# JuliaMeshless/WhatsThePoint.jl

Measured on AMD Instinct MI355X. Metric: Mpoints/sec per repel iter (k=21 KNN+force), higher is better.
Workload: dtype f32

## Files before the change

### whatsthepoint.jl_amd/csrc/wtp_cs2.hip

```cpp
#include "wtp_device.hpp"

namespace wtp {

#ifndef WTP_DIAG
#define WTP_DIAG 0
#endif
#define CS_STAMP(i)                                                 \
    if (WTP_DIAG) {                                                 \
        const unsigned long long t_ = __builtin_amdgcn_s_memtime(); \
        dt[i] += t_ - t_last;                                       \
        t_last = t_;                                                \
    }

constexpr int kCsThreads = 256;
constexpr int kCsSlab = 16;
constexpr int kCsMaxBX = 61;
constexpr int kCsMaxCells = (kCsMaxBX + 2) * kCsSlab;
constexpr int kCsMaskSteps = 12;
constexpr int kCsSU = 8;
constexpr int kCsPadBytes = 2 * kCsSU * 16;
constexpr int kCsMaxQ = 512;
constexpr int kCsMiss = 16;
constexpr int kCsRun = 2 * kCsSlab + 2 * 4 + 3;

struct CsMiss {
    uint32_t pa, ea, qoff;
    int32_t gslot, qid;
    float f, s, g2;
};

struct Cs2Smem {
    uint32_t hglobal[kCsMaxCells];
    uint16_t ls[kCsMaxCells + 4];
    uint16_t qpref[kCsMaxBX + 2];
    uint8_t qslab[kCsMaxQ];
    uint32_t wsum[4][64], wcnt[4][64], wown[2][64];
    int scan_tmp[kCsThreads / 64 + 1];
    int miss_n[kCsThreads / 64];
    CsMiss miss[kCsThreads / 64][kCsMiss];
    Acc acc[kCsThreads / 64];
};

struct CsAcc {
    float max_force, argmin_r;
    double sum_u, sum_u2;
    int32_t argmin_i, argmin_j, n_move;
};
__device__ inline float cs_step_point(const SearchArgs<float>& a, float s, float xi, float yi, float zi, float Fx, float Fy,
                                      float Fz, float& xo, float& yo, float& zo) {
    const float Fn = __builtin_amdgcn_sqrtf((Fx * Fx + Fy * Fy) + Fz * Fz);
    float al = __builtin_amdgcn_rcpf(Fn + 1.0e-30f);
// ... 10 lines not shown
}

__device__ inline void cs_acc_point(CsAcc& c, float force, float nd, float s, int32_t id, int32_t nn) {
    c.max_force = force > c.max_force ? force : c.max_force;
    const float rs = __builtin_amdgcn_rcpf(s), q0 = nd * rs;
    const double u = (double)__builtin_fmaf(__builtin_fmaf(-s, q0, nd), rs, q0);
    c.sum_u += u;
    c.sum_u2 += u * u;
    c.n_move += 1;
    if (nd < c.argmin_r || (nd == c.argmin_r && id < c.argmin_i)) {
        c.argmin_r = nd;
        c.argmin_i = id;
        c.argmin_j = nn;
    }
}

struct ForceCoefCs {
    float A, beta;
};
__device__ inline ForceCoefCs force_coef_cs(float beta, float u0) { return ForceCoefCs{u0 * u0, beta}; }

static size_t cs2_smem_bytes(int hcap) {
    return (size_t)hcap * 16 + kCsPadBytes + sizeof(Cs2Smem);
}

template <bool CH>
__global__ __launch_bounds__(kCsThreads, 4) void cs2_kernel(SearchArgs<float> a, int hcap, int BX) {
    if (a.stop && *a.stop) return;
    extern __shared__ __attribute__((aligned(16))) unsigned char smem_raw[];
    float4* pts = reinterpret_cast<float4*>(smem_raw);
    Cs2Smem* sm = reinterpret_cast<Cs2Smem*>(smem_raw + (size_t)hcap * 16 + kCsPadBytes);
    const int tid = threadIdx.x, lane = tid & 63;
    const int wave = __builtin_amdgcn_readfirstlane(tid >> 6);

    const Grid<float> g = *a.grid;
    const int K = a.k;
    const int HX = BX + 2, ncell = HX * kCsSlab;
    const int nbx = (g.n[0] + BX - 1) / BX, nby = (g.n[1] + 1) / 2, nbz = (g.n[2] + 1) / 2;
    const int nbricks = nbx * nby * nbz;
    CsAcc acc;
    acc.max_force = 0.f;
    acc.argmin_r = Lim<float>::inf();
    acc.sum_u = acc.sum_u2 = 0.0;
    acc.argmin_i = acc.argmin_j = -1;
    acc.n_move = 0;
    unsigned long long dt[16] = {0, 0, 0, 0, 0, 0, 0, 0, 0, 0, 0, 0, 0, 0, 0, 0};
// ... 47 lines not shown
            const int r = wave * 4 + j;
            const int gy = oy + (r & 3), gz = oz + (r >> 2);
            const bool row_ok = gy >= 0 && gy < g.n[1] && gz >= 0 && gz < g.n[2];
            vv[j] = a.cell_start[row_ok ? (gz * g.n[1] + gy) * g.n[0] + gxc : 0];
        }
    };
    auto load_points = [&](const int (&vv)[4], float4 (&pp)[4]) {
        const int last = a.n - 1;
#pragma unroll
        for (int j = 0; j < 4; ++j) {
            const int gs = __builtin_amdgcn_readfirstlane(vv[j]);
            const int len = __builtin_amdgcn_readlane(vv[j], HX < 63 ? HX : 63) - gs;
            const int i = gs + (lane < len ? lane : 0);
            pp[j] = a.snap[i < last ? i : last];
        }
    };

    auto skip_dead = [&](int& b, BrickPos& p) {
        while (a.brick_dead && b < b_end && b < a.brick_dead_cap && a.brick_dead[b]) {
            b += blk_per_group;
            advance(p);
        }
    };
    int brick = xcd * per + lane_blk;
    BrickPos pos = brick_pos(brick < nbricks ? brick : 0);
    skip_dead(brick, pos);
    BrickPos pos_next = pos;
    int next = brick;
    int v[4] = {0, 0, 0, 0};
    float4 pv[4];
    pv[0] = pv[1] = pv[2] = pv[3] = make_float4(0.f, 0.f, 0.f, 0.f);
    if (brick < b_end) {
        load_cells(pos, v);
        load_points(v, pv);
    }
    for (; brick < b_end; brick = next, pos = pos_next) {
        int bx, ox, oy, oz;
        origin(pos, bx, ox, oy, oz);
        next = brick + blk_per_group;
        advance(pos_next);
        skip_dead(next, pos_next);

        __builtin_amdgcn_s_setprio(0);
        __syncthreads();
        int vn[4] = {0, 0, 0, 0};
        if (next < b_end) load_cells(pos_next, vn);
// ... 320 lines not shown
            a.forces[gslot] = f;
            const bool has = nid != 0x7FFFFFFF;
            if (has) {
                const float nd = wsqrt(nd2);
                if (reaches_past_cover<float>(a, qp.x, qp.y, qp.z, lim)) atomicAdd(a.uncovered, 1);
                a.nn_dist[gslot] = nd;
                a.nn_id[gslot] = nid;
                cs_acc_point(acc, f, nd, s, qid, nid);
            }
            const unsigned long long mm = __ballot(!has);
            if (mm) {
                const int base_m = sm->miss_n[wave];
                if (!has) {
                    const int pos = base_m + (int)__popcll(mm & ((1ull << lane) - 1ull));
                    if (pos < kCsMiss) {
                        CsMiss e;
                        e.pa = pa_first;
                        e.ea = ea_all;
                        e.qoff = qoff;
                        e.gslot = gslot;
                        e.qid = qid;
                        e.f = f;
                        e.s = s;
                        e.g2 = safe_radius2(g, qp.x, qp.y, qp.z, cx, cy, cz, 1);
                        sm->miss[wave][pos] = e;
                    } else {
                        const int p2 = atomicAdd(a.fb_count, 1);
                        a.fb_list[p2] = gslot;
                    }
                }
                const int first = __ffsll((long long)mm) - 1;
                const int tot = base_m + (int)__popcll(mm);
                __builtin_amdgcn_wave_barrier();
                if (lane == first) sm->miss_n[wave] = tot < kCsMiss ? tot : kCsMiss;
                __builtin_amdgcn_wave_barrier();
            }
            CS_STAMP(4)
        }

        {
            const int nm = __builtin_amdgcn_readfirstlane(sm->miss_n[wave]);
            for (int m = 0; m < nm; ++m) {
                const CsMiss e = sm->miss[wave][m];
                const float4 qp = lds_pt(smem_raw, e.qoff);
                float bd = Lim<float>::inf();
                int32_t bi = 0x7FFFFFFF;
                for (uint32_t p = e.pa + (uint32_t)lane * 16u; p < e.ea; p += 64u * 16u) {
                    const float4 c = lds_pt(smem_raw, p);
                    const int32_t cid = w_to_id(c.w);
                    const float d = dist2<float>(qp.x, qp.y, qp.z, c.x, c.y, c.z);
                    if (cid != e.qid && lex_lt(d, cid, bd, bi)) {
                        bd = d;
                        bi = cid;
                    }
                }
#pragma unroll
                for (int dlt = 32; dlt >= 1; dlt >>= 1) {
                    const float od = __shfl_xor(bd, dlt, 64);
                    const int32_t oi = __shfl_xor(bi, dlt, 64);
                    if (lex_lt(od, oi, bd, bi)) {
                        bd = od;
                        bi = oi;
                    }
                }
                if (lane == 0) {
                    if (bi != 0x7FFFFFFF && bd <= e.g2) {
                        const float nd = wsqrt(bd);
                        if (reaches_past_cover<float>(a, qp.x, qp.y, qp.z, bd)) atomicAdd(a.uncovered, 1);
                        a.nn_dist[e.gslot] = nd;
                        a.nn_id[e.gslot] = bi;
                        cs_acc_point(acc, e.f, nd, e.s, e.qid, bi);
                    } else {
                        a.nn_dist[e.gslot] = bd;
                        a.nn_id[e.gslot] = bi == 0x7FFFFFFF ? -1 : bi;
                        const int pos = atomicAdd(a.nn_count, 1);
                        a.nn_list[pos] = e.gslot;
                    }
                }
            }
            if (WTP_DIAG) dt[14] += (unsigned long long)nm;
        }
        CS_STAMP(5)
    }
    if (WTP_DIAG && a.diag && lane == 0) {
        for (int i = 0; i < 15; ++i) atomicAdd(&a.diag[i], dt[i]);
        atomicAdd(&a.diag[15], 1ull);
    }
    __syncthreads();
    Acc full = acc_empty();
    full.max_force = (double)acc.max_force;
    full.sum_u = acc.sum_u;
    full.sum_u2 = acc.sum_u2;
    full.n_move = acc.n_move;
    if (acc.argmin_i >= 0) {
        full.argmin_r = (double)acc.argmin_r;
        full.argmin_i = acc.argmin_i;
        full.argmin_j = acc.argmin_j;
    }
    acc_block_reduce(full, sm->acc);
    if (tid == 0) acc_store(&a.partials[blockIdx.x], full);
}

__global__ void cs2_census_kernel(const int32_t* __restrict__ cell_start, const Grid<float>* __restrict__ gp, int BX,
                                  unsigned int* __restrict__ out ) {
    const Grid<float> g = *gp;
    const int nbx = (g.n[0] + BX - 1) / BX, nby = (g.n[1] + 1) / 2, nbz = (g.n[2] + 1) / 2;
    const int nbricks = nbx * nby * nbz;
    for (int brick = blockIdx.x * blockDim.x + threadIdx.x; brick < nbricks; brick += gridDim.x * blockDim.x) {
        const int bx = brick % nbx, by = (brick / nbx) % nby, bz = brick / (nbx * nby);
// ... 5 lines not shown
            if (gy < 0 || gy >= g.n[1] || gz < 0 || gz >= g.n[2]) continue;
            const int base = (gz * g.n[1] + gy) * g.n[0];
            H += cell_start[base + hx1 + 1] - cell_start[base + hx0];
            const bool own = ((r & 3) == 1 || (r & 3) == 2) && ((r >> 2) == 1 || (r >> 2) == 2);
            if (own) Q += cell_start[base + gx1 + 1] - cell_start[base + gx0];
        }
        if (Q == 0) continue;
        atomicAdd(&out[Q / 2 < 255 ? Q / 2 : 255], 1u);
        atomicAdd(&out[256 + (H / 8 < 255 ? H / 8 : 255)], 1u);
        atomicAdd(&out[512], 1u);
    }
}

int launch_cs2_census(wtp_ctx* ctx, int BX, unsigned int* d_out513) {
    WTP_HIP(ctx, hipMemsetAsync(d_out513, 0, 513 * sizeof(unsigned int), ctx->stream));
    hipLaunchKernelGGL(cs2_census_kernel, dim3(512), dim3(256), 0, ctx->stream, (const int32_t*)ctx->cell_start.p,
                       (const Grid<float>*)ctx->grid.p, BX, d_out513);
    WTP_HIP(ctx, hipGetLastError());
    return WTP_OK;
}

int cs2_max_bx() { return kCsMaxBX; }

constexpr int kNnFixBlocks = 512;
constexpr int kNnFixThreads = 1024;
__global__ __launch_bounds__(kNnFixThreads, 8) void cs2_nnfix_kernel(SearchArgs<float> a, int part_base) {
    if (a.stop && *a.stop) return;
    __shared__ Acc sacc[kNnFixThreads / 64];
    const Grid<float> g = *a.grid;
    const int n = *a.nn_count;
    const int lane = threadIdx.x & 63;
    const int wave_g = (blockIdx.x * kNnFixThreads + threadIdx.x) >> 6, nwaves = (gridDim.x * kNnFixThreads) >> 6;
    Acc acc = acc_empty();
    const int grp = lane >> 4, l16 = lane & 15;
    for (int i0 = wave_g * 4; i0 < n; i0 += nwaves * 4) {
        const int i = i0 + grp;
        const bool on = i < n;
        const int gslot = a.nn_list[on ? i : i0];
        const float4 qp = a.snap[gslot];
        const int32_t qid = w_to_id(qp.w);
        const int cx = cell_coord(g, qp.x, 0), cy = cell_coord(g, qp.y, 1), cz = cell_coord(g, qp.z, 2);
        float bd = a.nn_dist[gslot];
        int32_t bi = a.nn_id[gslot];
        bi = bi < 0 ? 0x7FFFFFFF : bi;
        auto gap = [&](float v, int axis, int c, int lo, int hi) {
            const float a0 = g.org[axis] + (float)(c + lo) * g.c, a1 = g.org[axis] + (float)(c + hi + 1) * g.c;
            float d = v < a0 ? a0 - v : (v > a1 ? v - a1 : 0.f);
            d -= g.margin;
            return d > 0.f ? d : 0.f;
        };
        for (int piece = l16; piece < 75; piece += 16) {
            const int r = piece / 3, seg = piece % 3;
            const int dz = r / 5 - 2, dy = r % 5 - 2;
            const bool inner = dz >= -1 && dz <= 1 && dy >= -1 && dy <= 1;
            if (inner && seg == 1) continue;
            const int gz = cz + dz, gy = cy + dy;
            if (gz < 0 || gz >= g.n[2] || gy < 0 || gy >= g.n[1]) continue;
            int xa = seg == 0 ? cx - 2 : (seg == 1 ? cx - 1 : cx + 2), xb = seg == 1 ? cx + 1 : xa;
            xa = xa < 0 ? 0 : xa;
            xb = xb > g.n[0] - 1 ? g.n[0] - 1 : xb;
            if (xa > xb) continue;
            const bool edge = xa == 0 || xb == g.n[0] - 1 || gy == 0 || gy == g.n[1] - 1 || gz == 0 || gz == g.n[2] - 1;
            if (!edge) {
                const float gx2 = gap(qp.x, 0, 0, xa, xb), gy2 = gap(qp.y, 1, gy, 0, 0), gz2 = gap(qp.z, 2, gz, 0, 0);
                if ((gx2 * gx2 + gy2 * gy2) + gz2 * gz2 > bd) continue;
            }
            const int base = (gz * g.n[1] + gy) * g.n[0];
            const int p1 = a.cell_start[base + xb + 1];
            for (int p = a.cell_start[base + xa]; p < p1; p += 4) {
                float4 c[4];
#pragma unroll
                for (int u = 0; u < 4; ++u) c[u] = a.snap[p + u < p1 ? p + u : p];
#pragma unroll
                for (int u = 0; u < 4; ++u) {
                    const int32_t cid = w_to_id(c[u].w);
                    const float d = dist2<float>(qp.x, qp.y, qp.z, c[u].x, c[u].y, c[u].z);
                    if (p + u < p1 && cid != qid && lex_lt(d, cid, bd, bi)) {
                        bd = d;
                        bi = cid;
                    }
                }
            }
        }
#pragma unroll
        for (int dlt = 8; dlt >= 1; dlt >>= 1) {
            const float od = __shfl_xor(bd, dlt, 64);
            const int32_t oi = __shfl_xor(bi, dlt, 64);
            if (lex_lt(od, oi, bd, bi)) {
                bd = od;
                bi = oi;
            }
        }
        if (l16 == 0 && on) {
            const float g2 = safe_radius2(g, qp.x, qp.y, qp.z, cx, cy, cz, 2);
            if (bi != 0x7FFFFFFF && bd <= g2) {
                const float s = a.spacing_pp ? a.spacing_pp[qid] : a.spacing_const;
                const float nd = wsqrt(bd);
                if (reaches_past_cover<float>(a, qp.x, qp.y, qp.z, bd)) atomicAdd(a.uncovered, 1);
                a.nn_dist[gslot] = nd;
                a.nn_id[gslot] = bi;
                acc_point<float>(acc, a.forces[gslot], nd, s, qid, bi);
            } else {
                const int pos = atomicAdd(a.fb_count, 1);
                a.fb_list[pos] = gslot;
            }
        }
    }
    acc_block_reduce(acc, sacc);
    if (threadIdx.x == 0) acc_store(&a.partials[part_base + blockIdx.x], acc);
}

constexpr int kBallThreads = 256;
constexpr int kBallBlocksMax = 3072;
constexpr int kBallRMax = 4;
#ifndef WTP_BALL_LANES
#define WTP_BALL_LANES 8
#endif
constexpr int kBallLanes = WTP_BALL_LANES;
constexpr int kBallPerWave = 64 / kBallLanes;
__global__ __launch_bounds__(kBallThreads, 6) void cs_ball_kernel(SearchArgs<float> a, const int32_t* __restrict__ list,
                                                               const int32_t* __restrict__ list_count,
                                                               int32_t* __restrict__ out_list, int32_t* __restrict__ out_count,
                                                               int part_base) {
    if (a.stop && *a.stop) return;
    __shared__ Acc sacc[kBallThreads / 64];
    const Grid<float> g = *a.grid;
    const int n = *list_count;
    const int K = a.k;
    const int lane = threadIdx.x & 63;
    const int grp = lane / kBallLanes, l16 = lane % kBallLanes;
    const int wave_g = (blockIdx.x * kBallThreads + threadIdx.x) >> 6, nwaves = (gridDim.x * kBallThreads) >> 6;
    const ForceCoef fc = force_coef(WTP_FORCE_CLIPPED_SPACING, a.beta, a.u0, 0.f);
    Acc acc = acc_empty();
// ... 170 lines not shown
    return WTP_OK;
}

int launch_cs2(wtp_ctx* ctx, SearchArgs<float>& a) {
    const int hcap = a.brick_hcap, BX = a.cs2_bx;
    if (hcap < 64 || hcap > 4096 || BX < 1 || BX > kCsMaxBX)
        return fail(ctx, WTP_ERR_STATE, "compact-support sweep launched without a brick geometry");
    const size_t smem = cs2_smem_bytes(hcap);
    const bool chunked = a.cs2_chunked != 0;
    const void* fn = chunked ? (const void*)cs2_kernel<true> : (const void*)cs2_kernel<false>;
    if (ctx->cs2_smem != smem || ctx->cs2_fn != fn) {
        WTP_HIP(ctx, hipFuncSetAttribute(fn, hipFuncAttributeMaxDynamicSharedMemorySize, (int)smem));
        int occ = 0;
        hipError_t e = chunked ? hipOccupancyMaxActiveBlocksPerMultiprocessor(&occ, cs2_kernel<true>, kCsThreads, smem)
                               : hipOccupancyMaxActiveBlocksPerMultiprocessor(&occ, cs2_kernel<false>, kCsThreads, smem);
        if (e != hipSuccess || occ < 1) occ = 1;
        ctx->cs2_occ = occ > 4 ? 4 : occ;
        ctx->cs2_smem = smem;
        ctx->cs2_fn = fn;
    }
    int gsz = ctx->sm_count * ctx->cs2_occ;
    gsz -= gsz % 8;
    if (gsz < 8) gsz = 8;
    if (chunked)
        hipLaunchKernelGGL(cs2_kernel<true>, dim3(gsz), dim3(kCsThreads), smem, ctx->stream, a, hcap, BX);
    else
        hipLaunchKernelGGL(cs2_kernel<false>, dim3(gsz), dim3(kCsThreads), smem, ctx->stream, a, hcap, BX);
    a.used_brick = gsz;
    WTP_HIP(ctx, hipGetLastError());
    return WTP_OK;
}

int launch_cs2_followup(wtp_ctx* ctx, SearchArgs<float>& a) {
    int blocks = (int)((a.n + 2047) / 2048);
    blocks = blocks < 8 ? 8 : (blocks > kNnFixBlocks ? kNnFixBlocks : blocks);
    hipLaunchKernelGGL(cs2_nnfix_kernel, dim3(blocks), dim3(kNnFixThreads), 0, ctx->stream, a, a.used_brick);
    a.used_brick += blocks;
    WTP_HIP(ctx, hipGetLastError());
    return WTP_OK;
}

}
```

### whatsthepoint.jl_amd/csrc/wtp_device.hpp

```cpp
#pragma once
#include "wtp_internal.hpp"

namespace wtp {

template <typename T> struct Lim;
template <> struct Lim<float> {
    static __device__ __host__ constexpr float inf() { return __builtin_huge_valf(); }
};
template <> struct Lim<double> {
    static __device__ __host__ constexpr double inf() { return __builtin_huge_val(); }
};

__device__ inline float wsqrt(float x) { return __builtin_sqrtf(x); }
__device__ inline double wsqrt(double x) { return __builtin_sqrt(x); }
__device__ inline float wfloor(float x) { return floorf(x); }
__device__ inline double wfloor(double x) { return floor(x); }
__device__ inline float wpow(float a, float b) { return powf(a, b); }
__device__ inline double wpow(double a, double b) { return pow(a, b); }

template <typename T>
__device__ inline T dist2(T ax, T ay, T az, T bx, T by, T bz) {
    T dx = ax - bx;
    T dy = ay - by;
    T dz = az - bz;
// ... 10 lines not shown
template <typename T>
__device__ inline int cell_coord(const Grid<T>& g, T v, int axis) {
    T f = wfloor((v - g.org[axis]) * g.inv_c);
    int c = (f > (T)0) ? ((f < (T)(g.n[axis] - 1)) ? (int)f : g.n[axis] - 1) : 0;
    return c;
}

template <typename T>
__device__ inline T safe_radius2(const Grid<T>& g, T qx, T qy, T qz, int cx, int cy, int cz, int r) {
    T best = Lim<T>::inf();
    const T q[3] = {qx, qy, qz};
    const int c[3] = {cx, cy, cz};
#pragma unroll
    for (int a = 0; a < 3; ++a) {
        if (a >= g.dim) break;
        T rel = q[a] - g.org[a];
        if (c[a] - r > 0) {
            T lo = rel - (T)(c[a] - r) * g.c;
            best = lo < best ? lo : best;
        }
        if (c[a] + r < g.n[a] - 1) {
            T hi = (T)(c[a] + r + 1) * g.c - rel;
            best = hi < best ? hi : best;
        }
    }
    if (best == Lim<T>::inf()) return best;
    best = best - g.margin;
    if (best < (T)0) best = (T)0;
    return best * best;
}

template <typename T>
__device__ inline T force_law(int kind, T beta, T u0, T gamma, T u) {
    T u2 = u * u;
    T d = u2 + beta;
    if (kind == WTP_FORCE_INVERSE_DISTANCE) return (T)1 / (d * d);
    if (kind == WTP_FORCE_SPACING_EQUILIBRIUM) return ((T)1 - u2) / (d * d);
    if (kind == WTP_FORCE_CLIPPED_SPACING) {
        T f = (u0 * u0 - u2) / (d * d);
        return f > (T)0 ? f : (T)0;
    }
    return ((T)1 - u2) / wpow(d, gamma);
}

template <typename T>
__device__ inline void fallback_dir(int64_t i, int64_t j, int dim, T out[3]) {
// ... 257 lines not shown
```

### whatsthepoint.jl_amd/csrc/wtp_generic.hip

```cpp
#include "wtp_device.hpp"

namespace wtp {

static constexpr int kThreads = 128;

template <typename T, int MODE>
__global__ __launch_bounds__(kThreads) void generic_kernel(SearchArgs<T> a, const int32_t* __restrict__ list,
                                                           const int32_t* __restrict__ list_count,
                                                           int all, int part_base) {
    if (a.stop && *a.stop) return;
    __shared__ Acc sm_acc[kThreads / 64];
    const Grid<T> g = *a.grid;
    const int nq = all ? a.n : *list_count;
    const int K = a.k;
    const bool skip_self = (MODE == 0) && !a.include_self;
    T bd[kGenericKMax];
    int32_t bi[kGenericKMax];
    int32_t bp[kGenericKMax];
    Acc acc = acc_empty();

    for (int qi = blockIdx.x * blockDim.x + threadIdx.x; qi < nq; qi += gridDim.x * blockDim.x) {
        const int slot = all ? qi : list[qi];
        const Pt<T> q = a.query[slot];
        const int32_t id = w_to_id(q.w);
        if (MODE == 1 && id < a.n_fixed) {
            a.out[slot] = q;
            a.forces[slot] = (T)0;
            a.nn_dist[slot] = Lim<T>::inf();
            a.nn_id[slot] = -1;
            continue;
        }
        const int cx = cell_coord(g, q.x, 0), cy = cell_coord(g, q.y, 1), cz = cell_coord(g, q.z, 2);
        int m = 0;
        for (int r = 1;; r *= 2) {
            m = 0;
            const int z0 = cz - r < 0 ? 0 : cz - r, z1 = cz + r > g.n[2] - 1 ? g.n[2] - 1 : cz + r;
// ... 260 lines not shown
```

### whatsthepoint.jl_amd/csrc/wtp_internal.hpp

```cpp
#pragma once
#include <hip/hip_runtime.h>
#include <stddef.h>
#include <stdint.h>
#include <functional>
#include <map>
#include <string>
#include <utility>
#include <vector>

#include "../../include/wtp.h"

namespace wtp {

template <typename T> struct PtOf;
template <> struct PtOf<float> { using type = float4; };
template <> struct PtOf<double> { using type = double4; };
template <typename T> using Pt = typename PtOf<T>::type;

using KnnStats = struct ::wtp_knn_stats;

template <typename F> inline auto by_dtype(int dtype, F&& f) { return dtype == WTP_F32 ? f(float{}) : f(double{}); }

__host__ __device__ inline float id_to_w(float, int32_t id) { return __builtin_bit_cast(float, id); }
__host__ __device__ inline double id_to_w(double, int32_t id) {
// ... 32 lines not shown
int brick_partials();
constexpr int kGenericKMax = 128;

constexpr double kGammaCap = 1.0;
constexpr double kGammaCapSweep = 0.96;
constexpr double kTnnFrac = 0.8;
constexpr double kRhoCs2 = 1.0;
constexpr double kRhoKsel = 1.2;
constexpr double kCapKsel = 40.0;
constexpr int kGridReuseMax = 7;

struct Partial {
    double max_force;
    double sum_u;
    double sum_u2;
    double argmin_r;
    int64_t argmin_i;
    int64_t argmin_j;
    int64_t n_move;
};

struct StepCounters {
    int32_t brick_handbacks, pad1_;
    int32_t nn_count, pad3_;
    int32_t wave_handbacks, pad5_;
    int32_t ball_count, pad7_;
    int32_t uncovered, pad9_[3];
    int32_t escaped, pad13_[3];
};
static_assert(sizeof(StepCounters) == 64 && offsetof(StepCounters, escaped) == 48, "16 words: the reduction zeroes exactly these");

struct RadCursor {
    unsigned long long arena_next;
    int32_t bricks_listed;
    int32_t dense_queries;
};
static_assert(sizeof(RadCursor) == 16, "wtp_radb.hip addresses these words by offset");

struct ForceParams {
    int32_t kind;
    double beta, u0, gamma;
};

template <typename T> struct SearchArgs {
    const Grid<T>* grid;
    const Pt<T>* snap;
    const int32_t* cell_start;
// ... 13 lines not shown
    T beta, u0, gamma;
    int32_t force_kind;
    int32_t n_fixed;
    Partial* partials;
    int32_t n_partials;
    int32_t used_brick, used_wave, used_generic;
    T radius2;
    int32_t* rad_counts;
    const int64_t* rad_offsets;
    int32_t rad_fill;
    int32_t* rad_tmp;
    uint8_t* rad_done;
    int32_t* rad_arena;
    int64_t* rad_arena_off;
    unsigned long long* rad_arena_pos;
    int64_t rad_arena_cap;
    int32_t* rad_bricks;
    int32_t rad_dense;
    int32_t* fb_list;
    int32_t* fb_count;
    int32_t* fb2_list;
    int32_t* fb2_count;
    int32_t* nn_list;
    int32_t* nn_count;
    int32_t* ball_list;
    int32_t* ball_count;
    const int32_t* stop;
    int32_t cover_axis;
    T cover_lo, cover_hi;
    T cover_lo3[3], cover_hi3[3];
    int32_t* uncovered;
    T gamma_cap;
    float cap_count;
    T tnn_frac;
    int32_t brick_hcap;
    int32_t cs2_bx;
    const uint8_t* brick_dead;
    int32_t brick_dead_cap;
    int32_t cs2_chunked;
    int32_t counters_cleared;
    int32_t fb_r0;
    int32_t ksel_bx;
    unsigned long long* diag;
};

struct DevBuf {
    void* p = nullptr;
// ... 341 lines not shown

inline int grid_for(int64_t n, int threads, int cap) {
    int64_t b = (n + threads - 1) / threads;
    if (b < 1) b = 1;
    return (int)(b > cap ? cap : b);
}
template <typename T> int launch_topology(wtp_ctx* ctx, SearchArgs<T>& a);
int launch_brick_sweep(wtp_ctx* ctx, SearchArgs<float>& a, bool cs);
template <typename T> int launch_brick_cs(wtp_ctx* ctx, SearchArgs<T>& a);
template <typename T> int launch_wave_topology(wtp_ctx* ctx, SearchArgs<T>& a, bool all);
template <typename T> int launch_wave_sweep(wtp_ctx* ctx, SearchArgs<T>& a, bool all);
template <typename T>
int launch_wave_radius_count(wtp_ctx* ctx, SearchArgs<T>& a, T r, int32_t* d_counts, const int32_t* list,
                             const int32_t* list_count);
template <typename T>
int launch_wave_radius_fill(wtp_ctx* ctx, SearchArgs<T>& a, T r, const int64_t* d_offsets, int32_t* d_idx,
                            const int32_t* list, const int32_t* list_count);
template <typename T> int launch_generic_topology(wtp_ctx* ctx, SearchArgs<T>& a, bool all);
template <typename T> int launch_query_knn(wtp_ctx* ctx, SearchArgs<T>& a, const T* d_xyz, int dim, Pt<T>* d_packed);
template <typename T> int launch_generic_sweep(wtp_ctx* ctx, SearchArgs<T>& a, bool all);
inline int total_partials() { return brick_partials() + kWavePartials + kGenericPartials; }
int launch_brick_radius(wtp_ctx* ctx, SearchArgs<float>& a);
int launch_cs2(wtp_ctx* ctx, SearchArgs<float>& a);
int launch_cs2_followup(wtp_ctx* ctx, SearchArgs<float>& a);
int debug_kd_steps(unsigned long long out[2]);
int launch_cs_ball(wtp_ctx* ctx, SearchArgs<float>& a, int32_t* rest_list, int32_t* rest_count);
int launch_cs2_census(wtp_ctx* ctx, int BX, unsigned int* d_out513);
int launch_cs2_dead(wtp_ctx* ctx, SearchArgs<float>& a, uint8_t* d_dead, int dead_cap);
int cs2_max_bx();
int launch_ksel_topology(wtp_ctx* ctx, SearchArgs<float>& a);
int launch_ksel_sweep(wtp_ctx* ctx, SearchArgs<float>& a);
int ksel_max_bx();
int ksel_kmax();
template <typename T>
int launch_radius_count(wtp_ctx* ctx, SearchArgs<T>& a, T r, int32_t* d_counts);
template <typename T>
int launch_radius_fill(wtp_ctx* ctx, SearchArgs<T>& a, T r, const int64_t* d_offsets,
                       int32_t* d_idx);
int launch_reduce_partials(wtp_ctx* ctx, const Partial* parts, int n_parts, int used_brick, int used_wave,
                           int used_generic, const int32_t* fb_count, const int32_t* uncovered,
                           const int32_t* escaped, wtp_step_stats* d_stats_slot);
template <typename T>
int launch_pca_normals(wtp_ctx* ctx, const T* d_xyz, int64_t n, int dim, const int32_t* d_rows, int k, T* d_out);
template <typename T>
int launch_minplus_batch(wtp_ctx* ctx, const int32_t* d_rows, const T* d_dist, int64_t n, int k, double g, double tol,
                         T* d_h0, T* d_h1, int first, int sweeps, unsigned long long* d_state);
size_t knn_stats_tmp_bytes(int64_t n);
template <typename T>
int launch_knn_stats(wtp_ctx* ctx, const T* d_dist, int64_t n, int k, const double* d_h, double h_const, int has_spacing,
                     double coord_radius, const int64_t* d_gid, T* d_nn_out, double* d_mean_out, void* d_tmp,
                     const KnnStats** d_result_out, const unsigned long long** d_bad_out);
int knn_stats_spacing(const void* h, double h_const, double coord_radius, const char** why);
// ... 84 lines not shown
```

### whatsthepoint.jl_amd/csrc/wtp_relax.hip

```cpp
#include <cstdlib>
#include <cstring>

#include "wtp_internal.hpp"

using namespace wtp;

#define WTP_API extern "C"

static double host_max(const void* v, int64_t n, int dtype) {
    double m = 0;
    if (dtype == WTP_F64) {
        const double* p = (const double*)v;
        for (int64_t i = 0; i < n; ++i) m = p[i] > m ? p[i] : m;
    } else {
        const float* p = (const float*)v;
        for (int64_t i = 0; i < n; ++i) m = p[i] > m ? p[i] : m;
    }
    return m;
}

static double spacing_law_max(const wtp_spacing_desc* s) {
    if (s->kind == WTP_SPACING_LOGLIKE) return s->p0;
    return s->p0 > s->p1 ? s->p0 : s->p1;
}
// ... 254 lines not shown
            if (route == SweepRoute::Cs2 && ball) {
                const int dead_cap = (int)(ctx->cell_start.cap / sizeof(int32_t) / 4 + 4096);
                rc = ensure(ctx, ctx->brick_dead, (size_t)dead_cap);
                if (!rc) rc = launch_cs2_dead(ctx, a, (uint8_t*)ctx->brick_dead.p, dead_cap);
                a.brick_dead = (const uint8_t*)ctx->brick_dead.p;
                a.brick_dead_cap = dead_cap;
            }
            if (!rc) rc = route == SweepRoute::Cs2 ? launch_cs2(ctx, a) : launch_brick_sweep(ctx, a, route == SweepRoute::Cs);
        }
        break;
    case SweepRoute::Cs64:
    case SweepRoute::Cs64Wave:
        sp = span_begin(ctx, 1);
        if constexpr (!f32) {
            rc = launch_brick_cs<double>(ctx, a);
            if (!rc && ball) rc = ball_pass(ctx, a);
        }
        break;
    }
    span_end(ctx, sp);
    if (rc) return rc;
    sp = span_begin(ctx, 2);
    if constexpr (f32) {
        if (route == SweepRoute::Cs2) rc = launch_cs2_followup(ctx, a);
        if (!rc && ball) rc = ball_pass(ctx, a);
    }
    if (!rc) rc = launch_generic_sweep<T>(ctx, a, false);
    span_end(ctx, sp);
    return rc;
}

template <typename T>
static HashBuild<T> relax_request(const wtp_ctx* ctx, const RelaxState& r, const Pt<T>* in, Pt<T>* out, int64_t n, int k,
                                  const HashView& view, bool keep_grid) {
    const RouteGrid g = route_grid(ctx, r);
    HashBuild<T> b(in, out, n, r.dim, k);
    b.rho_direct = g.rho;
    b.min_cell = g.min_cell;
    b.cell_scale = r.tune.scale;
    b.view = view;
    b.keep_grid = keep_grid;
    b.canonical = !r.tune.valid || r.route != SweepRoute::F64Ksel;
    b.box = r.tune.clipped ? (const double*)ctx->box_dev.p : nullptr;
    return b;
}

template <typename T> static int relax_rebuild(wtp_ctx* ctx) {
    RelaxState& r = ctx->relax;
// ... 80 lines not shown
    SearchArgs<T> a{};
    init_search(a, ctx, (const Pt<T>*)ctx->pts[r.bufS].p, (const Pt<T>*)ctx->pts[r.bufP].p, r.n, r.k, 1);
    a.out = (Pt<T>*)ctx->pts[o].p;
    a.forces = (T*)ctx->forces.p;
    a.nn_dist = (T*)ctx->nn_dist.p;
    a.nn_id = (int32_t*)ctx->nn_id.p;
    a.spacing_pp = r.spacing_kind != WTP_SPACING_CONSTANT ? (const T*)ctx->spacing_pp.p : nullptr;
    a.spacing_const = (T)r.spacing_const;
    a.alpha_lo = (T)r.alpha_lo;
    a.alpha_max = (T)r.alpha_max;
    a.beta = (T)r.force.beta;
    a.u0 = (T)r.force.u0;
    a.gamma = (T)r.force.gamma;
    a.force_kind = r.force.kind;
    a.n_fixed = (int32_t)r.n_fixed;
    a.partials = (Partial*)ctx->partials.p;
    a.n_partials = total_partials();
    StepCounters* counters = step_counters(ctx);
    a.fb_list = (int32_t*)ctx->fb_list.p;
    a.fb_count = &counters->brick_handbacks;
    a.fb2_list = (int32_t*)ctx->fb2_list.p;
    a.fb2_count = &counters->wave_handbacks;
    a.stop = ctx->stop_dev;
    a.nn_count = &counters->nn_count;
    const SweepRoute route = step_route(r, fresh);
    const bool ball = route_ball(r.route) && (!fresh || r.spacing_kind != WTP_SPACING_CONSTANT);
    if (ball || route == SweepRoute::Cs2) {
        if ((rc = ensure(ctx, ctx->nn_list, sizeof(int32_t) * (size_t)r.n))) return rc;
        if (sizeof(T) == 4) a.nn_list = (int32_t*)ctx->nn_list.p;
        if (ball) {
            a.ball_list = (int32_t*)ctx->nn_list.p;
            a.ball_count = &counters->ball_count;
        }
    }
    if ((rc = ensure(ctx, ctx->diag, 128))) return rc;
    a.diag = (unsigned long long*)ctx->diag.p;
    a.brick_hcap = route_cs(r.route) ? r.brick_hcap : (r.route == SweepRoute::Ksel ? r.tune.hcap : 0);
    a.cs2_bx = route_cs(r.route) ? r.cs2_bx : 0;
    a.cs2_chunked = (r.spacing_kind != WTP_SPACING_CONSTANT || r.cs2_rho > 1.6) ? 1 : 0;
    a.ksel_bx = r.route == SweepRoute::Ksel ? r.tune.bx : 0;
    if (r.route == SweepRoute::Ksel) a.cap_count = (float)ksel_cap_count(r.k);
    if (route == SweepRoute::Select || route == SweepRoute::Cs || route == SweepRoute::Cs2) {
        a.gamma_cap = (T)kGammaCapSweep;
        a.cap_count = (float)(4.18879 * kGammaCapSweep * kGammaCapSweep * kGammaCapSweep * ctx->rho * (a.k + 1) / 22.0);
    }
    if (route == SweepRoute::Cs64 || route == SweepRoute::Cs64Wave) a.gamma_cap = (T)kGammaCap;
    a.tnn_frac = (T)kTnnFrac;
    a.cover_axis = r.cover_axis;
    a.cover_lo = (T)r.cover_lo;
    a.cover_hi = (T)r.cover_hi;
    for (int ax = 0; ax < 3; ++ax) {
        a.cover_lo3[ax] = (T)r.cover_lo3[ax];
// ... 395 lines not shown
```

### whatsthepoint.jl_amd/csrc/wtp_wave.hip

```cpp
#include "wtp_device.hpp"

namespace wtp {

static constexpr int kWaves = 4;
static constexpr int kThreads = kWaves * 64;
static constexpr int kCap = 512;
static constexpr int kKeyRegs = kCap / 64;
static constexpr int kSurv = 256;

template <typename T> struct Bits;
template <> struct Bits<float> {
    using U = uint32_t;
    static __device__ U of(float v) { return __builtin_bit_cast(uint32_t, v); }
    static __device__ float back(U u) { return __builtin_bit_cast(float, u); }
    static constexpr U kInf = 0x7F800000u;
};
template <> struct Bits<double> {
    using U = uint64_t;
    static __device__ U of(double v) { return __builtin_bit_cast(uint64_t, v); }
    static __device__ double back(U u) { return __builtin_bit_cast(double, u); }
    static constexpr U kInf = 0x7FF0000000000000ull;
};

template <typename T, bool SWEEP> struct WaveSmem;
// ... 14 lines not shown
    int32_t id[kCap];
    T sd2[kSurv];
    int32_t sid[kSurv];
    T od2[kGenericKMax];
    int32_t oid[kGenericKMax];
};

__device__ inline int lane_id() { return __builtin_amdgcn_mbcnt_hi(~0u, __builtin_amdgcn_mbcnt_lo(~0u, 0)); }

template <typename T, int MODE>
__global__ __launch_bounds__(kThreads) void wave_kernel(SearchArgs<T> a, const int32_t* __restrict__ list,
                                                        const int32_t* __restrict__ list_count, int all,
                                                        int part_base) {
    if (a.stop && *a.stop) return;
    extern __shared__ __attribute__((aligned(16))) unsigned char smem_raw[];
    using U = typename Bits<T>::U;
    const int wave = threadIdx.x >> 6;
    const int lane = threadIdx.x & 63;
    using Smem = WaveSmem<T, MODE == 1>;
    Smem* sm = reinterpret_cast<Smem*>(smem_raw) + wave;
    Acc* sm_acc = reinterpret_cast<Acc*>(smem_raw + sizeof(Smem) * kWaves);
    const Grid<T> g = *a.grid;
    const int nq = all ? a.n : *list_count;
    const int K = a.k;
    const bool skip_self = (MODE == 0) && !a.include_self;
    Acc acc = acc_empty();
    const int wave_global = blockIdx.x * kWaves + wave;
    const int wave_stride = gridDim.x * kWaves;

    for (int qi = wave_global; qi < nq; qi += wave_stride) {
        const int slot = all ? qi : list[qi];
        const Pt<T> q = a.query[slot];
        const int32_t id = w_to_id(q.w);
        if (MODE == 1 && id < a.n_fixed) {
            if (lane == 0) {
                a.out[slot] = q;
                a.forces[slot] = (T)0;
                a.nn_dist[slot] = Lim<T>::inf();
                a.nn_id[slot] = -1;
            }
            continue;
        }
        const int cx = cell_coord(g, q.x, 0), cy = cell_coord(g, q.y, 1), cz = cell_coord(g, q.z, 2);
        int m = 0;
        bool overflow = false;
        int Kq = K;
// ... 483 lines not shown
```

Before: 12710.

## Fold nearest-neighbour fixup into cs2 sweep with per-wave pending lists

Removes the separate cs2_nnfix kernel launch and resolves uncertified nearest-neighbour misses inside the cs2 kernel. A miss first gets a wider search over the LDS-resident halo (±2 x-columns) with a box-based safe radius, then unresolved ones go to per-wave pending lists that are processed after the brick loop with the global 5x5 shell scan. The global nn_count atomic is replaced by per-wave slices, and the wave and generic kernels gain early exits for blocks with no work. This saves a launch and a global atomic, but it adds tail work and register pressure to the main kernel and overflow goes to the fallback list.

```diff
diff --git a/whatsthepoint.jl_amd/csrc/wtp_cs2.hip b/whatsthepoint.jl_amd/csrc/wtp_cs2.hip
--- a/whatsthepoint.jl_amd/csrc/wtp_cs2.hip
+++ b/whatsthepoint.jl_amd/csrc/wtp_cs2.hip
@@ -26,7 +26,8 @@
 struct CsMiss {
     uint32_t pa, ea, qoff;
     int32_t gslot, qid;
-    float f, s, g2;
+    float f, s;
+    uint32_t cxy, czh;
 };
 
 struct Cs2Smem {
@@ -83,6 +84,80 @@
 
 static size_t cs2_smem_bytes(int hcap) {
     return (size_t)hcap * 16 + kCsPadBytes + sizeof(Cs2Smem);
+}
+
+__device__ inline void cs_wave_nearest(const unsigned char* smem_raw, uint32_t pa, uint32_t ea, const float4& qp, int32_t qid,
+                                       int lane, float& bd, int32_t& bi) {
+    for (uint32_t p = pa + (uint32_t)lane * 16u; p < ea; p += 64u * 16u) {
+        const float4 c = lds_pt(smem_raw, p);
+        const int32_t cid = w_to_id(c.w);
+        const float d = dist2<float>(qp.x, qp.y, qp.z, c.x, c.y, c.z);
+        if (cid != qid && lex_lt(d, cid, bd, bi)) {
+            bd = d;
+            bi = cid;
+        }
+    }
+#pragma unroll
+    for (int dlt = 32; dlt >= 1; dlt >>= 1) {
+        const float od = __shfl_xor(bd, dlt, 64);
+        const int32_t oi = __shfl_xor(bi, dlt, 64);
+        if (lex_lt(od, oi, bd, bi)) {
+            bd = od;
+            bi = oi;
+        }
+    }
+}
+
+__device__ inline void cs_shell_nearest(const SearchArgs<float>& a, const Grid<float>& g, const float4& qp, int32_t qid, int cx,
+                                        int cy, int cz, int l16, float& bd, int32_t& bi) {
+    auto gap = [&](float v, int axis, int c, int lo, int hi) {
+        const float a0 = g.org[axis] + (float)(c + lo) * g.c, a1 = g.org[axis] + (float)(c + hi + 1) * g.c;
+        float d = v < a0 ? a0 - v : (v > a1 ? v - a1 : 0.f);
+        d -= g.margin;
+        return d > 0.f ? d : 0.f;
+    };
+    for (int piece = l16; piece < 75; piece += 16) {
+        const int r = piece / 3, seg = piece % 3;
+        const int dz = r / 5 - 2, dy = r % 5 - 2;
+        const bool inner = dz >= -1 && dz <= 1 && dy >= -1 && dy <= 1;
+        if (inner && seg == 1) continue;
+        const int gz = cz + dz, gy = cy + dy;
+        if (gz < 0 || gz >= g.n[2] || gy < 0 || gy >= g.n[1]) continue;
+        int xa = seg == 0 ? cx - 2 : (seg == 1 ? cx - 1 : cx + 2), xb = seg == 1 ? cx + 1 : xa;
+        xa = xa < 0 ? 0 : xa;
+        xb = xb > g.n[0] - 1 ? g.n[0] - 1 : xb;
+        if (xa > xb) continue;
+        const bool edge = xa == 0 || xb == g.n[0] - 1 || gy == 0 || gy == g.n[1] - 1 || gz == 0 || gz == g.n[2] - 1;
+        if (!edge) {
+            const float gx2 = gap(qp.x, 0, 0, xa, xb), gy2 = gap(qp.y, 1, gy, 0, 0), gz2 = gap(qp.z, 2, gz, 0, 0);
+            if ((gx2 * gx2 + gy2 * gy2) + gz2 * gz2 > bd) continue;
+        }
+        const int base = (gz * g.n[1] + gy) * g.n[0];
+        const int p1 = a.cell_start[base + xb + 1];
+        for (int p = a.cell_start[base + xa]; p < p1; p += 4) {
+            float4 c[4];
+#pragma unroll
+            for (int u = 0; u < 4; ++u) c[u] = a.snap[p + u < p1 ? p + u : p];
+#pragma unroll
+            for (int u = 0; u < 4; ++u) {
+                const int32_t cid = w_to_id(c[u].w);
+                const float d = dist2<float>(qp.x, qp.y, qp.z, c[u].x, c[u].y, c[u].z);
+                if (p + u < p1 && cid != qid && lex_lt(d, cid, bd, bi)) {
+                    bd = d;
+                    bi = cid;
+                }
+            }
+        }
+    }
+#pragma unroll
+    for (int dlt = 8; dlt >= 1; dlt >>= 1) {
+        const float od = __shfl_xor(bd, dlt, 64);
+        const int32_t oi = __shfl_xor(bi, dlt, 64);
+        if (lex_lt(od, oi, bd, bi)) {
+            bd = od;
+            bi = oi;
+        }
+    }
 }
 
 template <bool CH>
@@ -176,6 +251,9 @@
             advance(p);
         }
     };
+    const int pend_base = ((int)blockIdx.x * (kCsThreads / 64) + wave) * a.nn_cap;
+    int pend_n = 0;
+
     int brick = xcd * per + lane_blk;
     BrickPos pos = brick_pos(brick < nbricks ? brick : 0);
     skip_dead(brick, pos);
@@ -542,7 +620,8 @@
                         e.qid = qid;
                         e.f = f;
                         e.s = s;
-                        e.g2 = safe_radius2(g, qp.x, qp.y, qp.z, cx, cy, cz, 1);
+                        e.cxy = (uint32_t)cx | ((uint32_t)cy << 16);
+                        e.czh = (uint32_t)cz | ((uint32_t)(hx * kCsSlab + cellp) << 16);
                         sm->miss[wave][pos] = e;
                     } else {
                         const int p2 = atomicAdd(a.fb_count, 1);
@@ -565,36 +644,39 @@
                 const float4 qp = lds_pt(smem_raw, e.qoff);
                 float bd = Lim<float>::inf();
                 int32_t bi = 0x7FFFFFFF;
-                for (uint32_t p = e.pa + (uint32_t)lane * 16u; p < e.ea; p += 64u * 16u) {
-                    const float4 c = lds_pt(smem_raw, p);
-                    const int32_t cid = w_to_id(c.w);
-                    const float d = dist2<float>(qp.x, qp.y, qp.z, c.x, c.y, c.z);
-                    if (cid != e.qid && lex_lt(d, cid, bd, bi)) {
-                        bd = d;
-                        bi = cid;
-                    }
-                }
-#pragma unroll
-                for (int dlt = 32; dlt >= 1; dlt >>= 1) {
-                    const float od = __shfl_xor(bd, dlt, 64);
-                    const int32_t oi = __shfl_xor(bi, dlt, 64);
-                    if (lex_lt(od, oi, bd, bi)) {
-                        bd = od;
-                        bi = oi;
-                    }
-                }
-                if (lane == 0) {
-                    if (bi != 0x7FFFFFFF && bd <= e.g2) {
+                cs_wave_nearest(smem_raw, e.pa, e.ea, qp, e.qid, lane, bd, bi);
+                const int cxq = (int)(e.cxy & 0xFFFFu), cyq = (int)(e.cxy >> 16), czq = (int)(e.czh & 0xFFFFu);
+                const float g2 = safe_radius2(g, qp.x, qp.y, qp.z, cxq, cyq, czq, 1);
+                bool cert = __builtin_amdgcn_readfirstlane((int)(bi != 0x7FFFFFFF && bd <= g2)) != 0;
+                if (!cert) {
+                    const int hxq = (int)(e.czh >> 20), hyq = (int)((e.czh >> 16) & 3u), hzq = (int)((e.czh >> 18) & 3u);
+                    const int x0 = hxq - 2 < 0 ? 0 : hxq - 2, x1 = hxq + 2 > HX - 1 ? HX - 1 : hxq + 2;
+                    cs_wave_nearest(smem_raw, (uint32_t)sm->ls[x0 * kCsSlab] * 16u, (uint32_t)sm->ls[(x1 + 1) * kCsSlab] * 16u, qp,
+                                    e.qid, lane, bd, bi);
+                    const int lo[3] = {hxq - x0, hyq, hzq}, hi[3] = {x1 - hxq, 3 - hyq, 3 - hzq};
+                    const float g2b = safe_radius2_box(g, qp.x, qp.y, qp.z, cxq, cyq, czq, lo, hi);
+                    cert = __builtin_amdgcn_readfirstlane((int)(bi != 0x7FFFFFFF && bd <= g2b)) != 0;
+                }
+                if (cert) {
+                    if (lane == 0) {
                         const float nd = wsqrt(bd);
                         if (reaches_past_cover<float>(a, qp.x, qp.y, qp.z, bd)) atomicAdd(a.uncovered, 1);
                         a.nn_dist[e.gslot] = nd;
                         a.nn_id[e.gslot] = bi;
                         cs_acc_point(acc, e.f, nd, e.s, e.qid, bi);
-                    } else {
+                    }
+                    continue;
+                }
+                const bool room = pend_n < a.nn_cap;
+                pend_n = __builtin_amdgcn_readfirstlane(pend_n + (room ? 1 : 0));
+                if (lane == 0) {
+                    if (room) {
                         a.nn_dist[e.gslot] = bd;
                         a.nn_id[e.gslot] = bi == 0x7FFFFFFF ? -1 : bi;
-                        const int pos = atomicAdd(a.nn_count, 1);
-                        a.nn_list[pos] = e.gslot;
+                        a.nn_list[pend_base + pend_n - 1] = e.gslot;
+                    } else {
+                        const int pos = atomicAdd(a.fb_count, 1);
+                        a.fb_list[pos] = e.gslot;
                     }
                 }
             }
@@ -605,6 +687,36 @@
     if (WTP_DIAG && a.diag && lane == 0) {
         for (int i = 0; i < 15; ++i) atomicAdd(&a.diag[i], dt[i]);
         atomicAdd(&a.diag[15], 1ull);
+    }
+    {
+        const int np = pend_n;
+        if (np > 0) __threadfence_block();
+        const int grp = lane >> 4, l16 = lane & 15;
+        for (int i0 = 0; i0 < np; i0 += 4) {
+            const bool on = i0 + grp < np;
+            const int gslot = a.nn_list[pend_base + (on ? i0 + grp : i0)];
+            const float4 qp = a.snap[gslot];
+            const int32_t qid = w_to_id(qp.w);
+            const int cx = cell_coord(g, qp.x, 0), cy = cell_coord(g, qp.y, 1), cz = cell_coord(g, qp.z, 2);
+            float bd = a.nn_dist[gslot];
+            int32_t bi = a.nn_id[gslot];
+            bi = bi < 0 ? 0x7FFFFFFF : bi;
+            cs_shell_nearest(a, g, qp, qid, cx, cy, cz, l16, bd, bi);
+            if (l16 == 0 && on) {
+                const float g2 = safe_radius2(g, qp.x, qp.y, qp.z, cx, cy, cz, 2);
+                if (bi != 0x7FFFFFFF && bd <= g2) {
+                    const float s = a.spacing_pp ? a.spacing_pp[qid] : a.spacing_const;
+                    const float nd = wsqrt(bd);
+                    if (reaches_past_cover<float>(a, qp.x, qp.y, qp.z, bd)) atomicAdd(a.uncovered, 1);
+                    a.nn_dist[gslot] = nd;
+                    a.nn_id[gslot] = bi;
+                    cs_acc_point(acc, a.forces[gslot], nd, s, qid, bi);
+                } else {
+                    const int pos = atomicAdd(a.fb_count, 1);
+                    a.fb_list[pos] = gslot;
+                }
+            }
+        }
     }
     __syncthreads();
     Acc full = acc_empty();
@@ -656,93 +768,7 @@
 
 int cs2_max_bx() { return kCsMaxBX; }
 
-constexpr int kNnFixBlocks = 512;
-constexpr int kNnFixThreads = 1024;
-__global__ __launch_bounds__(kNnFixThreads, 8) void cs2_nnfix_kernel(SearchArgs<float> a, int part_base) {
-    if (a.stop && *a.stop) return;
-    __shared__ Acc sacc[kNnFixThreads / 64];
-    const Grid<float> g = *a.grid;
-    const int n = *a.nn_count;
-    const int lane = threadIdx.x & 63;
-    const int wave_g = (blockIdx.x * kNnFixThreads + threadIdx.x) >> 6, nwaves = (gridDim.x * kNnFixThreads) >> 6;
-    Acc acc = acc_empty();
-    const int grp = lane >> 4, l16 = lane & 15;
-    for (int i0 = wave_g * 4; i0 < n; i0 += nwaves * 4) {
-        const int i = i0 + grp;
-        const bool on = i < n;
-        const int gslot = a.nn_list[on ? i : i0];
-        const float4 qp = a.snap[gslot];
-        const int32_t qid = w_to_id(qp.w);
-        const int cx = cell_coord(g, qp.x, 0), cy = cell_coord(g, qp.y, 1), cz = cell_coord(g, qp.z, 2);
-        float bd = a.nn_dist[gslot];
-        int32_t bi = a.nn_id[gslot];
-        bi = bi < 0 ? 0x7FFFFFFF : bi;
-        auto gap = [&](float v, int axis, int c, int lo, int hi) {
-            const float a0 = g.org[axis] + (float)(c + lo) * g.c, a1 = g.org[axis] + (float)(c + hi + 1) * g.c;
-            float d = v < a0 ? a0 - v : (v > a1 ? v - a1 : 0.f);
-            d -= g.margin;
-            return d > 0.f ? d : 0.f;
-        };
-        for (int piece = l16; piece < 75; piece += 16) {
-            const int r = piece / 3, seg = piece % 3;
-            const int dz = r / 5 - 2, dy = r % 5 - 2;
-            const bool inner = dz >= -1 && dz <= 1 && dy >= -1 && dy <= 1;
-            if (inner && seg == 1) continue;
-            const int gz = cz + dz, gy = cy + dy;
-            if (gz < 0 || gz >= g.n[2] || gy < 0 || gy >= g.n[1]) continue;
-            int xa = seg == 0 ? cx - 2 : (seg == 1 ? cx - 1 : cx + 2), xb = seg == 1 ? cx + 1 : xa;
-            xa = xa < 0 ? 0 : xa;
-            xb = xb > g.n[0] - 1 ? g.n[0] - 1 : xb;
-            if (xa > xb) continue;
-            const bool edge = xa == 0 || xb == g.n[0] - 1 || gy == 0 || gy == g.n[1] - 1 || gz == 0 || gz == g.n[2] - 1;
-            if (!edge) {
-                const float gx2 = gap(qp.x, 0, 0, xa, xb), gy2 = gap(qp.y, 1, gy, 0, 0), gz2 = gap(qp.z, 2, gz, 0, 0);
-                if ((gx2 * gx2 + gy2 * gy2) + gz2 * gz2 > bd) continue;
-            }
-            const int base = (gz * g.n[1] + gy) * g.n[0];
-            const int p1 = a.cell_start[base + xb + 1];
-            for (int p = a.cell_start[base + xa]; p < p1; p += 4) {
-                float4 c[4];
-#pragma unroll
-                for (int u = 0; u < 4; ++u) c[u] = a.snap[p + u < p1 ? p + u : p];
-#pragma unroll
-                for (int u = 0; u < 4; ++u) {
-                    const int32_t cid = w_to_id(c[u].w);
-                    const float d = dist2<float>(qp.x, qp.y, qp.z, c[u].x, c[u].y, c[u].z);
-                    if (p + u < p1 && cid != qid && lex_lt(d, cid, bd, bi)) {
-                        bd = d;
-                        bi = cid;
-                    }
-                }
-            }
-        }
-#pragma unroll
-        for (int dlt = 8; dlt >= 1; dlt >>= 1) {
-            const float od = __shfl_xor(bd, dlt, 64);
-            const int32_t oi = __shfl_xor(bi, dlt, 64);
-            if (lex_lt(od, oi, bd, bi)) {
-                bd = od;
-                bi = oi;
-            }
-        }
-        if (l16 == 0 && on) {
-            const float g2 = safe_radius2(g, qp.x, qp.y, qp.z, cx, cy, cz, 2);
-            if (bi != 0x7FFFFFFF && bd <= g2) {
-                const float s = a.spacing_pp ? a.spacing_pp[qid] : a.spacing_const;
-                const float nd = wsqrt(bd);
-                if (reaches_past_cover<float>(a, qp.x, qp.y, qp.z, bd)) atomicAdd(a.uncovered, 1);
-                a.nn_dist[gslot] = nd;
-                a.nn_id[gslot] = bi;
-                acc_point<float>(acc, a.forces[gslot], nd, s, qid, bi);
-            } else {
-                const int pos = atomicAdd(a.fb_count, 1);
-                a.fb_list[pos] = gslot;
-            }
-        }
-    }
-    acc_block_reduce(acc, sacc);
-    if (threadIdx.x == 0) acc_store(&a.partials[part_base + blockIdx.x], acc);
-}
+size_t cs2_wave_list_min(const wtp_ctx* ctx) { return (size_t)ctx->sm_count * 4 * (kCsThreads / 64) * kCsMiss; }
 
 constexpr int kBallThreads = 256;
 constexpr int kBallBlocksMax = 3072;
@@ -959,6 +985,9 @@
     int gsz = ctx->sm_count * ctx->cs2_occ;
     gsz -= gsz % 8;
     if (gsz < 8) gsz = 8;
+    const int64_t waves = (int64_t)gsz * (kCsThreads / 64);
+    if (!a.nn_list || a.nn_len < waves * kCsMiss) return fail(ctx, WTP_ERR_STATE, "compact-support sweep launched without its waves' lists");
+    a.nn_cap = (int)(a.nn_len / waves);
     if (chunked)
         hipLaunchKernelGGL(cs2_kernel<true>, dim3(gsz), dim3(kCsThreads), smem, ctx->stream, a, hcap, BX);
     else
@@ -968,13 +997,4 @@
     return WTP_OK;
 }
 
-int launch_cs2_followup(wtp_ctx* ctx, SearchArgs<float>& a) {
-    int blocks = (int)((a.n + 2047) / 2048);
-    blocks = blocks < 8 ? 8 : (blocks > kNnFixBlocks ? kNnFixBlocks : blocks);
-    hipLaunchKernelGGL(cs2_nnfix_kernel, dim3(blocks), dim3(kNnFixThreads), 0, ctx->stream, a, a.used_brick);
-    a.used_brick += blocks;
-    WTP_HIP(ctx, hipGetLastError());
-    return WTP_OK;
-}
-
-}
+}
diff --git a/whatsthepoint.jl_amd/csrc/wtp_device.hpp b/whatsthepoint.jl_amd/csrc/wtp_device.hpp
--- a/whatsthepoint.jl_amd/csrc/wtp_device.hpp
+++ b/whatsthepoint.jl_amd/csrc/wtp_device.hpp
@@ -56,6 +56,31 @@
         if (c[a] + r < g.n[a] - 1) {
             T hi = (T)(c[a] + r + 1) * g.c - rel;
             best = hi < best ? hi : best;
+        }
+    }
+    if (best == Lim<T>::inf()) return best;
+    best = best - g.margin;
+    if (best < (T)0) best = (T)0;
+    return best * best;
+}
+
+template <typename T>
+__device__ inline T safe_radius2_box(const Grid<T>& g, T qx, T qy, T qz, int cx, int cy, int cz, const int (&lo)[3],
+                                     const int (&hi)[3]) {
+    T best = Lim<T>::inf();
+    const T q[3] = {qx, qy, qz};
+    const int c[3] = {cx, cy, cz};
+#pragma unroll
+    for (int a = 0; a < 3; ++a) {
+        if (a >= g.dim) break;
+        T rel = q[a] - g.org[a];
+        if (c[a] - lo[a] > 0) {
+            T l = rel - (T)(c[a] - lo[a]) * g.c;
+            best = l < best ? l : best;
+        }
+        if (c[a] + hi[a] < g.n[a] - 1) {
+            T h = (T)(c[a] + hi[a] + 1) * g.c - rel;
+            best = h < best ? h : best;
         }
     }
     if (best == Lim<T>::inf()) return best;
diff --git a/whatsthepoint.jl_amd/csrc/wtp_generic.hip b/whatsthepoint.jl_amd/csrc/wtp_generic.hip
--- a/whatsthepoint.jl_amd/csrc/wtp_generic.hip
+++ b/whatsthepoint.jl_amd/csrc/wtp_generic.hip
@@ -12,6 +12,10 @@
     __shared__ Acc sm_acc[kThreads / 64];
     const Grid<T> g = *a.grid;
     const int nq = all ? a.n : *list_count;
+    if (MODE == 1 && (int)(blockIdx.x * blockDim.x) >= nq) {
+        if (threadIdx.x == 0) acc_store(&a.partials[part_base + blockIdx.x], acc_empty());
+        return;
+    }
     const int K = a.k;
     const bool skip_self = (MODE == 0) && !a.include_self;
     T bd[kGenericKMax];
diff --git a/whatsthepoint.jl_amd/csrc/wtp_internal.hpp b/whatsthepoint.jl_amd/csrc/wtp_internal.hpp
--- a/whatsthepoint.jl_amd/csrc/wtp_internal.hpp
+++ b/whatsthepoint.jl_amd/csrc/wtp_internal.hpp
@@ -78,7 +78,7 @@
 
 struct StepCounters {
     int32_t brick_handbacks, pad1_;
-    int32_t nn_count, pad3_;
+    int32_t pad2_, pad3_;
     int32_t wave_handbacks, pad5_;
     int32_t ball_count, pad7_;
     int32_t uncovered, pad9_[3];
@@ -138,7 +138,8 @@
     int32_t* fb2_list;
     int32_t* fb2_count;
     int32_t* nn_list;
-    int32_t* nn_count;
+    int64_t nn_len;
+    int32_t nn_cap;
     int32_t* ball_list;
     int32_t* ball_count;
     const int32_t* stop;
@@ -526,12 +527,12 @@
 inline int total_partials() { return brick_partials() + kWavePartials + kGenericPartials; }
 int launch_brick_radius(wtp_ctx* ctx, SearchArgs<float>& a);
 int launch_cs2(wtp_ctx* ctx, SearchArgs<float>& a);
-int launch_cs2_followup(wtp_ctx* ctx, SearchArgs<float>& a);
 int debug_kd_steps(unsigned long long out[2]);
 int launch_cs_ball(wtp_ctx* ctx, SearchArgs<float>& a, int32_t* rest_list, int32_t* rest_count);
 int launch_cs2_census(wtp_ctx* ctx, int BX, unsigned int* d_out513);
 int launch_cs2_dead(wtp_ctx* ctx, SearchArgs<float>& a, uint8_t* d_dead, int dead_cap);
 int cs2_max_bx();
+size_t cs2_wave_list_min(const wtp_ctx* ctx);
 int launch_ksel_topology(wtp_ctx* ctx, SearchArgs<float>& a);
 int launch_ksel_sweep(wtp_ctx* ctx, SearchArgs<float>& a);
 int ksel_max_bx();
diff --git a/whatsthepoint.jl_amd/csrc/wtp_relax.hip b/whatsthepoint.jl_amd/csrc/wtp_relax.hip
--- a/whatsthepoint.jl_amd/csrc/wtp_relax.hip
+++ b/whatsthepoint.jl_amd/csrc/wtp_relax.hip
@@ -300,8 +300,7 @@
     if (rc) return rc;
     sp = span_begin(ctx, 2);
     if constexpr (f32) {
-        if (route == SweepRoute::Cs2) rc = launch_cs2_followup(ctx, a);
-        if (!rc && ball) rc = ball_pass(ctx, a);
+        if (ball) rc = ball_pass(ctx, a);
     }
     if (!rc) rc = launch_generic_sweep<T>(ctx, a, false);
     span_end(ctx, sp);
@@ -428,12 +427,15 @@
     a.fb2_list = (int32_t*)ctx->fb2_list.p;
     a.fb2_count = &counters->wave_handbacks;
     a.stop = ctx->stop_dev;
-    a.nn_count = &counters->nn_count;
     const SweepRoute route = step_route(r, fresh);
     const bool ball = route_ball(r.route) && (!fresh || r.spacing_kind != WTP_SPACING_CONSTANT);
     if (ball || route == SweepRoute::Cs2) {
-        if ((rc = ensure(ctx, ctx->nn_list, sizeof(int32_t) * (size_t)r.n))) return rc;
-        if (sizeof(T) == 4) a.nn_list = (int32_t*)ctx->nn_list.p;
+        const size_t len = (size_t)r.n > cs2_wave_list_min(ctx) ? (size_t)r.n : cs2_wave_list_min(ctx);
+        if ((rc = ensure(ctx, ctx->nn_list, sizeof(int32_t) * len))) return rc;
+        if constexpr (sizeof(T) == 4) {
+            a.nn_list = (int32_t*)ctx->nn_list.p;
+            a.nn_len = (int64_t)len;
+        }
         if (ball) {
             a.ball_list = (int32_t*)ctx->nn_list.p;
             a.ball_count = &counters->ball_count;
diff --git a/whatsthepoint.jl_amd/csrc/wtp_wave.hip b/whatsthepoint.jl_amd/csrc/wtp_wave.hip
--- a/whatsthepoint.jl_amd/csrc/wtp_wave.hip
+++ b/whatsthepoint.jl_amd/csrc/wtp_wave.hip
@@ -60,6 +60,10 @@
     Acc* sm_acc = reinterpret_cast<Acc*>(smem_raw + sizeof(Smem) * kWaves);
     const Grid<T> g = *a.grid;
     const int nq = all ? a.n : *list_count;
+    if (MODE == 1 && (int)blockIdx.x * kWaves >= nq) {
+        if (threadIdx.x == 0) acc_store(&a.partials[part_base + blockIdx.x], acc_empty());
+        return;
+    }
     const int K = a.k;
     const bool skip_self = (MODE == 0) && !a.include_self;
     Acc acc = acc_empty();
```

Measured after the change: 12530. 0.986x the previous value.
